# GuanLab/seekmer

Measured on AMD Instinct MI355X. Metric: paired reads/sec mapped+quantified, higher is better.
Workload: dtype u64+f64; 1 GPU; configs[1]: synthetic ~190k-tx index (stand-in for ENSEMBL GRCh38 cDNA), 10000000 2x100bp synthetic pairs per GPU, map+classes+EM to the reference stop rule; transcripts=190402, kmer_slots=134217728, units_per_gpu=10000000, read_len=100, paired=True, classes=851072, class_map_rows=4208693, parallelism=reads sharded x1, RCCL all-reduce f64[T] per EM step, rccl_ranks=0

## Files before the change

### seekmer_amd/csrc/skm_abi.hip

```cpp
#include "../../include/seekmer_hip.h"
#include "skm_kernels.h"
#include "skm_pool.h"

#include <dlfcn.h>
#include <algorithm>
#include <cstdarg>
#include <cstdio>
#include <cstdlib>
#include <cstring>
#include <chrono>
#include <condition_variable>
#include <atomic>
#include <deque>
#include <functional>
#include <map>
#include <memory>
#include <unordered_map>
#include <mutex>
#include <thread>
#include <numeric>
#include <string>
#include <utility>
#include <vector>

// ... 218 lines not shown
struct skm_quant {
    ~skm_quant()
    {
        (void)hipSetDevice(device);
        if (stream) (void)hipStreamSynchronize(stream);
    }
    int device = 0;
    PoolStream stream;
    PoolTimingEvent ev[2];
    PoolEvent chunk_ev[2];
    PoolPinned pinned;
    std::mutex mu;
    int64_t n_tx = 0, n_classes = 0, n_ids = 0, n_rows = 0;
    DBuf<int64_t> cls_offset, row_start, tx_row;
    DBuf<int32_t> ids, tx_cls, row_tx, perm;
    DBuf<double> cls_count, cls_count_saved, inner, row_sum;
    DBuf<double> eff_len, x0, x1, acc, part_max;
    DBuf<unsigned int> part_flags, arrivals;
    DBuf<unsigned long long> ctl, cum;
    DBuf<unsigned int> tile_total;
    DBuf<double> x_start, boot_out;
    struct Batch {
        DBuf<double> cls_count, inner, row_sum, x0, x1, part_max;
        DBuf<unsigned int> part_flags;
        DBuf<unsigned long long> ctl, mgr;
        DBuf<double> counts_all;
        DBuf<double> totals;
        DBuf<int64_t> iters;
    } batch;
    struct Tiles {
        DBuf<int64_t> tile_tx, tile_cls, cls_pair, tx_pair;
        DBuf<int32_t> tx_list, cls_list, tx_label, tx_tile, cls_tile;
        DBuf<uint16_t> cls_tx, tx_cls;
        DBuf<double> x2, step_max;
        DBuf<unsigned int> step_flags;
        struct Residual {
            int64_t n_classes = 0, n_ids = 0, n_rows = 0;
            DBuf<int64_t> cls_offset, row_start, tx_row;
            DBuf<int32_t> ids, cls_src, row_tx, tx_cls;
            DBuf<double> cls_count, inner, row_sum;
            bool built = false;
        } residual;
        bool built = false;
        int64_t n_tiles = 0, n_oversize = 0;
    } tiles;
    double n_total = 0;
    bool n_total_reduced = false;
    void *comm = nullptr;
    int rank = 0, world = 1;
    double t_em_ns = 0, iters_total = 0, launches = 0;
};

struct skm_comm {
    int device = 0;
    void *comm = nullptr;
    int rank = 0, world = 1;
};

extern "C" const char *skm_last_error(void) { return g_error.c_str(); }

extern "C" int skm_device_count(int *count)
{
    if (!count) return fail(SKM_ERR_ARG, "count is NULL");
    int n = 0;
    hipError_t e = hipGetDeviceCount(&n);
    if (e != hipSuccess || n <= 0) {
        *count = 0;
// ... 2233 lines not shown
    HIP_TRY(pool_stream_acquire(q->stream.out()));
    for (auto &e : q->ev) HIP_TRY(pool_event_acquire(e.out(), true));
    for (auto &e : q->chunk_ev) HIP_TRY(pool_event_acquire(e.out(), false));
    HIP_TRY(pool_pinned_acquire((void **)q->pinned.out()));
    const size_t C = (size_t)std::max<int64_t>(n_classes, 1), M = (size_t)std::max<int64_t>(n_ids, 1);
    const size_t T = (size_t)std::max<int64_t>(n_tx, 1);
    const size_t R = (size_t)quant_rows_upper_bound(n_tx, n_ids);
    SKM_TRY(q->cls_offset.ensure(C + 1));
    SKM_TRY(q->cls_count.ensure(C));
    SKM_TRY(q->inner.ensure(C));
    SKM_TRY(q->ids.ensure(M));
    SKM_TRY(q->perm.ensure(C));
    SKM_TRY(q->tx_cls.ensure(M));
    SKM_TRY(q->tx_row.ensure(T + 1));
    SKM_TRY(q->row_start.ensure(R + 1));
    SKM_TRY(q->row_tx.ensure(R));
    SKM_TRY(q->row_sum.ensure(R));
    SKM_TRY(q->eff_len.ensure(T));
    SKM_TRY(q->x0.ensure(T));
    SKM_TRY(q->x1.ensure(T));
    SKM_TRY(q->acc.ensure(T));
    SKM_TRY(q->ctl.ensure(16));
    SKM_TRY(q->part_max.ensure(EM_FINAL_BLOCKS));
    SKM_TRY(q->part_flags.ensure(EM_FINAL_BLOCKS));
    SKM_TRY(q->arrivals.ensure(T));
    HIP_TRY(hipMemsetAsync(q->arrivals.p, 0, T * sizeof(unsigned int), q->stream));
    if (em_tiles_possible(several_ranks)) {
        auto &t = q->tiles;
        SKM_TRY(t.tile_tx.ensure(T + 2)); SKM_TRY(t.tile_cls.ensure(T + 2));
        SKM_TRY(t.cls_pair.ensure(C + 1)); SKM_TRY(t.tx_pair.ensure(T + 1));
        SKM_TRY(t.tx_list.ensure(T)); SKM_TRY(t.cls_list.ensure(C));
        SKM_TRY(t.tx_label.ensure(T)); SKM_TRY(t.tx_tile.ensure(T)); SKM_TRY(t.cls_tile.ensure(C));
        SKM_TRY(t.cls_tx.ensure(M)); SKM_TRY(t.tx_cls.ensure(M));
        SKM_TRY(t.x2.ensure(T));
    }
    STALE_CHECK("quant_alloc exit");
    return SKM_OK;
}

QuantBuild quant_build_view(skm_quant *q)
{
    QuantBuild b{};
    b.n_tx = q->n_tx;
    b.n_classes = q->n_classes;
    b.n_ids = q->n_ids;
    b.cls_offset = q->cls_offset.p;
    b.ids = q->ids.p;
    b.cls_count = q->cls_count.p;
    b.tx_cls = q->tx_cls.p;
    b.tx_row = q->tx_row.p;
    b.row_start = q->row_start.p;
    b.row_tx = q->row_tx.p;
    b.n_rows_cap = (int64_t)q->row_tx.cap;
    if (q->tiles.x2.p) {
        auto &t = q->tiles;
        b.tile_tx = t.tile_tx.p; b.tile_cls = t.tile_cls.p;
        b.tx_list = t.tx_list.p; b.cls_list = t.cls_list.p;
        b.cls_pair = t.cls_pair.p; b.tx_pair = t.tx_pair.p;
        b.tile_cls_tx = t.cls_tx.p; b.tile_tx_cls = t.tx_cls.p;
        b.tx_label = t.tx_label.p; b.tx_tile = t.tx_tile.p; b.cls_tile = t.cls_tile.p;
    }
    return b;
}

int quant_finish_setup(skm_quant *q, const ClassTable *table, int64_t units_seen = -1)
{
    STALE_CHECK("quant_finish_setup");
    QuantBuild b = quant_build_view(q);
    b.first_seen_bound = units_seen > 0 ? units_seen : 0;
    const int64_t rows = quant_setup(table, b, q->perm.p, q->stream);
    if (rows < 0) return fail(SKM_ERR_HIP, "building the class views failed (%lld): %s", (long long)rows, quant_setup_failure());
    q->n_rows = rows;
    if (b.tile_tx) {
        q->tiles.built = true;
        q->tiles.n_tiles = b.tile_info[0];
        q->tiles.n_oversize = b.tile_info[1];
        if (q->tiles.n_tiles > 0) {
            SKM_TRY(q->tiles.step_max.ensure((size_t)(EM_CHUNK_MAX * q->tiles.n_tiles)));
            SKM_TRY(q->tiles.step_flags.ensure((size_t)(EM_CHUNK_MAX * q->tiles.n_tiles)));
        }
        if (q->tiles.n_oversize > 0 && q->tiles.n_tiles > 0) {
            auto &r = q->tiles.residual;
            int64_t counts[3] = {0, 0, 0};
            if (quant_residual_count(b, counts, q->stream))
                return fail(SKM_ERR_HIP, "sizing the residual EM problem failed: %s", quant_setup_failure());
            r.n_classes = counts[0]; r.n_ids = counts[1]; r.n_rows = counts[2];
            SKM_TRY(r.cls_offset.ensure((size_t)r.n_classes + 1)); SKM_TRY(r.ids.ensure((size_t)std::max<int64_t>(r.n_ids, 1)));
            SKM_TRY(r.cls_src.ensure((size_t)std::max<int64_t>(r.n_classes, 1)));
            SKM_TRY(r.row_start.ensure((size_t)r.n_rows + 1)); SKM_TRY(r.row_tx.ensure((size_t)std::max<int64_t>(r.n_rows, 1)));
            SKM_TRY(r.tx_cls.ensure((size_t)std::max<int64_t>(r.n_ids, 1))); SKM_TRY(r.tx_row.ensure((size_t)q->n_tx + 1));
            SKM_TRY(r.cls_count.ensure((size_t)std::max<int64_t>(r.n_classes, 1)));
            SKM_TRY(r.inner.ensure((size_t)std::max<int64_t>(r.n_classes, 1)));
            SKM_TRY(r.row_sum.ensure((size_t)std::max<int64_t>(r.n_rows, 1)));
            QuantResidual out{};
            out.n_classes = r.n_classes; out.n_ids = r.n_ids; out.n_rows = r.n_rows;
            out.cls_offset = r.cls_offset.p; out.ids = r.ids.p; out.cls_src = r.cls_src.p;
            out.row_start = r.row_start.p; out.row_tx = r.row_tx.p; out.tx_cls = r.tx_cls.p; out.tx_row = r.tx_row.p;
            if (quant_residual_build(b, out, q->stream))
                return fail(SKM_ERR_HIP, "building the residual EM problem failed: %s", quant_setup_failure());
            r.built = true;
        }
    }
    return SKM_OK;
}

struct Rccl {
    void *lib = nullptr;
    int (*GetUniqueId)(void *) = nullptr;
    int (*AllReduce)(const void *, void *, size_t, int, int, void *, hipStream_t) = nullptr;
    int (*CommDestroy)(void *) = nullptr;
    int (*CommCount)(void *, int *) = nullptr;
    const char *(*GetErrorString)(int) = nullptr;
// ... 61 lines not shown
    p.x[1] = q->x1.p;
    p.acc = q->acc.p;
    p.n_total = q->n_total;
    p.rel_tol = rel_tol;
    p.x_floor = x_floor;
    p.ctl = q->ctl.p;
    p.part_max = q->part_max.p;
    p.part_flags = q->part_flags.p;
    p.max_iters = max_iters;
    p.fixed_iters = fixed_iters;
    static const bool unfused = getenv("SKM_EM_UNFUSED") != nullptr;
    p.fused = q->comm || unfused ? 0 : 1;
    p.arrivals = q->arrivals.p;
    return p;
}

bool em_uses_tiles(const skm_quant *q)
{
    return em_tiles_possible(q->comm != nullptr) && q->tiles.built && q->tiles.n_tiles > 0 &&
           (q->tiles.n_oversize == 0 || q->tiles.residual.built);
}

constexpr int CTL_WORD_TILE_FAULT = 4;
int em_run_tiles(skm_quant *q, const EmProblem &p, int64_t chunk, int64_t *iters_out)
{
    auto &t = q->tiles;
    EmTiles tl{};
    tl.n_tiles = t.n_tiles;
    tl.tile_tx = t.tile_tx.p; tl.tile_cls = t.tile_cls.p;
    tl.tx_list = t.tx_list.p; tl.cls_list = t.cls_list.p;
    tl.cls_pair = t.cls_pair.p; tl.tx_pair = t.tx_pair.p;
    tl.cls_tx = t.cls_tx.p; tl.tx_cls = t.tx_cls.p;
    tl.step_max = t.step_max.p; tl.step_flags = t.step_flags.p;
    double *const x[3] = {q->x0.p, q->x1.p, t.x2.p};
    const bool mixed = t.n_oversize > 0;
    EmProblem pr = p;
    if (mixed) {
        auto &r = t.residual;
        pr.n_classes = r.n_classes; pr.n_rows = r.n_rows;
        pr.cls_offset = r.cls_offset.p; pr.ids = r.ids.p; pr.cls_count = r.cls_count.p; pr.inner = r.inner.p;
        pr.row_start = r.row_start.p; pr.row_tx = r.row_tx.p; pr.tx_cls = r.tx_cls.p; pr.tx_row = r.tx_row.p;
        pr.row_sum = r.row_sum.p;
        pr.fused = 1;
        pr.extra_max = t.step_max.p; pr.extra_flags = t.step_flags.p; pr.n_extra = t.n_tiles;
        launch_permute_f64(q->cls_count.p, r.cls_src.p, r.n_classes, r.cls_count.p, false, q->stream);
    }
    int64_t queued = 0;
    auto enqueue_chunk = [&](int slot) -> int {
        launch_em_local_chunk(p, tl, x[queued % 3], x[(queued + 1) % 3], (int)chunk, true, q->stream);
        if (mixed) {
            pr.extra_first = queued * chunk;
            for (int64_t i = 0, k = queued * chunk; i < chunk; ++i, ++k) {
                launch_em_inner(pr, (int)(k & 1), i > 0, k, q->stream);
                launch_em_rows_finalize(pr, (int)(k & 1), q->stream);
            }
            launch_em_decide(pr, (queued + 1) * chunk, q->stream);
            q->launches += 2 * chunk + 2;
        } else {
            launch_em_local_decide(p, tl, queued * chunk, (int)chunk, q->stream);
            q->launches += 2;
        }
        ++queued;
        HIP_TRY(hipGetLastError());
        HIP_TRY(hipMemcpyAsync(q->pinned + 8 * slot, q->ctl.p, 8 * sizeof(unsigned long long),
                               hipMemcpyDeviceToHost, q->stream));
        HIP_TRY(hipEventRecord(q->chunk_ev[slot], q->stream));
        return SKM_OK;
    };
    unsigned long long ctl[8] = {0};
    SKM_TRY(enqueue_chunk(0));
    int64_t last = 0;
    for (int slot = 0;; slot ^= 1, ++last) {
        SKM_TRY(enqueue_chunk(slot ^ 1));
        HIP_TRY(hipEventSynchronize(q->chunk_ev[slot]));
        memcpy(ctl, q->pinned + 8 * slot, sizeof(ctl));
        if (ctl[0]) break;
    }
    if (ctl[CTL_WORD_TILE_FAULT]) {
        HIP_TRY(hipStreamSynchronize(q->stream));
        return fail(SKM_ERR_STATE, "a component tile exceeds the tile capacity: the class views of this handle are damaged");
    }
    const int64_t steps = (int64_t)ctl[1], into = steps - last * chunk;
    double *const result = (steps & 1) ? q->x1.p : q->x0.p;
    if (into == chunk && !mixed) {
        if (x[(last + 1) % 3] != result)
            HIP_TRY(hipMemcpyAsync(result, x[(last + 1) % 3], q->n_tx * 8, hipMemcpyDeviceToDevice, q->stream));
    } else {
        launch_em_local_chunk(p, tl, x[last % 3], result, (int)into, false, q->stream);
        q->launches += 1;
        HIP_TRY(hipGetLastError());
    }
    HIP_TRY(hipEventRecord(q->ev[1], q->stream));
    HIP_TRY(hipEventSynchronize(q->ev[1]));
    float ms = 0;
    HIP_TRY(hipEventElapsedTime(&ms, q->ev[0], q->ev[1]));
    q->t_em_ns += ms * 1e6;
    q->iters_total += (double)steps;
    if (iters_out) *iters_out = steps;
    if (ctl[3]) return fail(SKM_ERR_UNDEFINED, "no abundance above x_floor: numpy raises on max() of an empty selection");
    return SKM_OK;
}

int em_run(skm_quant *q, double rel_tol, double x_floor, int64_t max_iters, int64_t fixed_iters,
           int64_t *iters_out, int64_t chunk_steps = 16)
{
    double n_total = q->n_total;
    if (q->comm && !q->n_total_reduced) {
        HIP_TRY(hipMemcpyAsync(q->acc.p, &n_total, 8, hipMemcpyHostToDevice, q->stream));
        NCCL_TRY(g_rccl.AllReduce(q->acc.p, q->acc.p, 1, NCCL_FLOAT64, NCCL_SUM, q->comm, q->stream));
        HIP_TRY(hipMemcpyAsync(&n_total, q->acc.p, 8, hipMemcpyDeviceToHost, q->stream));
        HIP_TRY(hipStreamSynchronize(q->stream));
    }
    EmProblem p = em_problem(q, rel_tol, x_floor, max_iters, fixed_iters);
    p.n_total = n_total;
    HIP_TRY(hipMemsetAsync(q->ctl.p, 0, 16 * 8, q->stream));
    int64_t k = 0;
    const int64_t chunk = fixed_iters > 0 ? std::min<int64_t>(fixed_iters, chunk_steps) : chunk_steps;
    HIP_TRY(hipEventRecord(q->ev[0], q->stream));
    if (em_uses_tiles(q) && chunk <= EM_CHUNK_MAX) return em_run_tiles(q, p, chunk, iters_out);
    static const bool unfused_rows = getenv("SKM_EM_UNFUSED") != nullptr;
    auto enqueue_chunk = [&](int slot) -> int {
        for (int64_t i = 0; i < chunk; ++i, ++k) {
            launch_em_inner(p, (int)(k & 1), i > 0, k, q->stream);
            if (q->comm) {
// ... 778 lines not shown
```

### seekmer_amd/csrc/skm_em.hip

```cpp
#include "skm_kernels.h"

namespace skm {

enum { CTL_DONE = 0, CTL_ITERS = 1, CTL_UNDEFINED = 3, CTL_TILE_FAULT = 4 };

__device__ bool em_evaluate(const EmProblem &p, int n_parts, int64_t steps_done, bool publish);

__global__ void __launch_bounds__(256)
em_inner_kernel(EmProblem p, int parity, int eval_parts, int64_t steps_done)
{
    const int64_t c_first = blockIdx.x * (int64_t)blockDim.x + threadIdx.x;
    int64_t begin_first = 0, end_first = 0;
    double count_first = 1.0;
    if (c_first < p.n_classes) {
        begin_first = p.cls_offset[c_first];
        end_first = p.cls_offset[c_first + 1];
        count_first = p.cls_count[c_first];
    }
    if (eval_parts > 0 && blockIdx.x == 0) {
        if (p.ctl[CTL_DONE]) return;
        if (em_evaluate(p, eval_parts, steps_done, true)) return;
    } else if (p.ctl[CTL_DONE]) {
        return;
    }
// ... 223 lines not shown
    const int wave = threadIdx.x >> 6;
    if ((threadIdx.x & 63) == 0) { s_max[wave] = m; s_flags[wave] = f; }
    __syncthreads();
    if (threadIdx.x == 0) {
        for (int w = 0; w < 4; ++w) { m = s_max[w] > m ? s_max[w] : m; f |= s_flags[w]; }
        bool done, undefined = false;
        if (p.fixed_iters > 0) {
            done = steps_done >= p.fixed_iters;
        } else if (!(f & 1u)) {
            undefined = true;
            done = true;
        } else {
            done = (f & 2u) || !(m > p.rel_tol);
            if (p.max_iters > 0 && steps_done >= p.max_iters) done = true;
        }
        if (publish) {
            if (undefined) p.ctl[CTL_UNDEFINED] = 1;
            p.ctl[CTL_ITERS] = (unsigned long long)steps_done;
            p.ctl[CTL_DONE] = done ? 1ULL : 0ULL;
        }
        s_done = done ? 1 : 0;
    }
    __syncthreads();
    return s_done != 0;
}

__global__ void __launch_bounds__(256)
em_decide_kernel(EmProblem p, int n_parts, int64_t steps_done)
{
    if (p.ctl[CTL_DONE]) return;
    em_evaluate(p, n_parts, steps_done, true);
}

__global__ void __launch_bounds__(256)
em_local_chunk_kernel(EmProblem p, EmTiles tl, const double *x_in, double *x_out, int n_steps, int check_done)
{
    static_assert(EM_TILE_TX <= 8 * 32, "a lane group of the row phase takes at most eight transcripts");
    if (check_done && p.ctl[CTL_DONE]) return;
    __shared__ double s_x[2][EM_TILE_TX];
    __shared__ double s_eff[EM_TILE_TX];
    __shared__ double s_inner[EM_TILE_CLASSES];
    __shared__ double s_count[EM_TILE_CLASSES];
    __shared__ double s_max[EM_CHUNK_MAX][4];
    __shared__ unsigned int s_flags[EM_CHUNK_MAX][4];
    __shared__ int32_t s_tx[EM_TILE_TX];
    __shared__ uint16_t s_cls_tx[EM_TILE_PAIRS], s_tx_cls[EM_TILE_PAIRS];
    __shared__ uint16_t s_cls_off[EM_TILE_CLASSES + 1], s_tx_off[EM_TILE_TX + 1];
    const int64_t tile = blockIdx.x;
    const int64_t tx0 = tl.tile_tx[tile], cls0 = tl.tile_cls[tile];
    const int n_tx = (int)(tl.tile_tx[tile + 1] - tx0), n_cls = (int)(tl.tile_cls[tile + 1] - cls0);
    const int64_t cp0 = tl.cls_pair[cls0], tp0 = tl.tx_pair[tx0];
    const int n_pairs = (int)(tl.cls_pair[cls0 + n_cls] - cp0);
    if (n_tx > EM_TILE_TX || n_cls > EM_TILE_CLASSES || n_pairs > EM_TILE_PAIRS || n_tx < 0 || n_cls < 0 || n_pairs < 0) {
        if (threadIdx.x == 0) { p.ctl[CTL_TILE_FAULT] = 1; p.ctl[CTL_DONE] = 1; }
        return;
    }
    const int tid = threadIdx.x;
    for (int j = tid; j < n_pairs; j += 256) {
        s_cls_tx[j] = tl.cls_tx[cp0 + j];
        s_tx_cls[j] = tl.tx_cls[tp0 + j];
    }
    for (int k = tid; k <= n_cls; k += 256) {
        s_cls_off[k] = (uint16_t)(tl.cls_pair[cls0 + k] - cp0);
        if (k < n_cls) s_count[k] = p.cls_count[tl.cls_list[cls0 + k]];
    }
    for (int i = tid; i <= n_tx; i += 256) {
        s_tx_off[i] = (uint16_t)(tl.tx_pair[tx0 + i] - tp0);
        if (i < n_tx) {
            const int32_t t = tl.tx_list[tx0 + i];
            s_tx[i] = t;
            s_x[0][i] = x_in[t];
            s_eff[i] = p.eff_len[t];
        }
    }
    __syncthreads();
    const int sub = tid & 7, wave = tid >> 6;
    for (int step = 0; step < n_steps; ++step) {
        const double *x = s_x[step & 1];
        double *x_new = s_x[(step & 1) ^ 1];
        for (int k = tid; k < n_cls; k += 256) {
            const int end = s_cls_off[k + 1];
            double s = 0.0;
            for (int j = s_cls_off[k]; j < end; ++j) s += x[s_cls_tx[j]];
            s_inner[k] = s / s_count[k];
        }
        __syncthreads();
        double local_max = 0.0;
        unsigned int flags = 0;
        double my_a = 0.0, my_xt = 0.0;
        int my_i = -1, turn = 0;
        for (int i = tid >> 3; i < n_tx; i += 32, ++turn) {
            const double xt = x[i];
            const int end = s_tx_off[i + 1];
            int begin = s_tx_off[i];
            double a = 0.0;
            do {
                const int row_end = min(begin + EM_ROW_CAP, end);
                double s = 0.0;
                for (int e = begin + sub; e < row_end; e += 8) s += xt / s_inner[s_tx_cls[e]];
                s += __shfl_xor(s, 4, 8);
                s += __shfl_xor(s, 2, 8);
                s += __shfl_xor(s, 1, 8);
                a += s;
                begin = row_end;
            } while (begin < end);
            if (turn == sub) { my_a = a; my_xt = xt; my_i = i; }
        }
        if (my_i >= 0) {
            double v = my_a / s_eff[my_i] / p.n_total;
            if (v != v) v = 0.0;
            x_new[my_i] = v;
            if (v > p.x_floor) {
                const double change = fabs(v - my_xt) / v;
                if (change != change) flags |= 2u;
                else if (change > local_max) local_max = change;
                flags |= 1u;
            }
        }
        for (int d = 32; d > 0; d >>= 1) {
            const double o = __shfl_xor(local_max, d, 64);
            local_max = o > local_max ? o : local_max;
            flags |= __shfl_xor(flags, d, 64);
        }
        if ((tid & 63) == 0) { s_max[step][wave] = local_max; s_flags[step][wave] = flags; }
        __syncthreads();
    }
    const double *x = s_x[n_steps & 1];
    for (int i = tid; i < n_tx; i += 256) x_out[s_tx[i]] = x[i];
    if (tid < n_steps) {
        double m = s_max[tid][0];
        unsigned int f = s_flags[tid][0];
        for (int w = 1; w < 4; ++w) { m = s_max[tid][w] > m ? s_max[tid][w] : m; f |= s_flags[tid][w]; }
        tl.step_max[tid * tl.n_tiles + tile] = m;
        tl.step_flags[tid * tl.n_tiles + tile] = f;
    }
}

__global__ void __launch_bounds__(64 * EM_CHUNK_MAX)
em_local_decide_kernel(EmProblem p, EmTiles tl, int64_t first_step, int n_steps)
{
    if (p.ctl[CTL_DONE]) return;
    __shared__ double s_max[EM_CHUNK_MAX];
    __shared__ unsigned int s_flags[EM_CHUNK_MAX];
    const int step = threadIdx.x >> 6, lane = threadIdx.x & 63;
    if (step < n_steps) {
        double m = 0.0;
        unsigned int f = 0;
        const double *__restrict__ step_max = tl.step_max + step * tl.n_tiles;
        const unsigned int *__restrict__ step_flags = tl.step_flags + step * tl.n_tiles;
        int64_t b = lane;
        for (; b + 7 * 64 < tl.n_tiles; b += 8 * 64) {
            double o[8];
            unsigned int g[8];
#pragma unroll
            for (int k = 0; k < 8; ++k) { o[k] = step_max[b + 64 * k]; g[k] = step_flags[b + 64 * k]; }
#pragma unroll
            for (int k = 0; k < 8; ++k) { m = o[k] > m ? o[k] : m; f |= g[k]; }
        }
        for (; b < tl.n_tiles; b += 64) {
            const double o = step_max[b];
            m = o > m ? o : m;
// ... 277 lines not shown
    if (blocks < 1) blocks = 1;
    if (blocks > EM_FINAL_BLOCKS) blocks = EM_FINAL_BLOCKS;
    return (int)blocks;
}

void launch_em_inner(const EmProblem &p, int parity, bool judge_previous, int64_t steps_done, hipStream_t stream)
{
    hipLaunchKernelGGL(em_inner_kernel, dim3(chip_grid(p.n_classes, 256)), dim3(256), 0, stream, p, parity,
                       judge_previous ? em_final_blocks(p) : 0, steps_done);
}

void launch_em_decide(const EmProblem &p, int64_t steps_done, hipStream_t stream)
{
    hipLaunchKernelGGL(em_decide_kernel, dim3(1), dim3(256), 0, stream, p, em_final_blocks(p), steps_done);
}

void launch_em_rows(const EmProblem &p, int parity, hipStream_t stream)
{
    hipLaunchKernelGGL(em_rows_kernel, dim3(chip_grid(p.n_rows, 32)), dim3(256), 0, stream, p, parity);
}

void launch_em_rows_finalize(const EmProblem &p, int parity, hipStream_t stream)
{
    hipLaunchKernelGGL(em_rows_finalize_kernel<false>, dim3((unsigned)em_final_blocks(p)), dim3(256), 0, stream, p, parity);
}

void launch_em_rows_acc(const EmProblem &p, int parity, hipStream_t stream)
{
    EmProblem fused = p;
    fused.fused = 1;
    hipLaunchKernelGGL(em_rows_finalize_kernel<true>, dim3((unsigned)em_final_blocks(fused)), dim3(256), 0, stream, p, parity);
}

void launch_em_local_chunk(const EmProblem &p, const EmTiles &tiles, const double *x_in, double *x_out, int n_steps,
                           bool check_done, hipStream_t stream)
{
    if (tiles.n_tiles <= 0 || n_steps <= 0) return;
    hipLaunchKernelGGL(em_local_chunk_kernel, dim3((unsigned)tiles.n_tiles), dim3(256), 0, stream, p, tiles, x_in, x_out,
                       std::min(n_steps, EM_CHUNK_MAX), check_done ? 1 : 0);
}

void launch_em_local_decide(const EmProblem &p, const EmTiles &tiles, int64_t first_step, int n_steps, hipStream_t stream)
{
    hipLaunchKernelGGL(em_local_decide_kernel, dim3(1), dim3(64 * EM_CHUNK_MAX), 0, stream, p, tiles, first_step,
                       std::min(n_steps, EM_CHUNK_MAX));
}

void launch_em_rows_to_acc(const EmProblem &p, hipStream_t stream)
{
    hipLaunchKernelGGL(em_rows_to_acc_kernel, dim3(chip_grid(p.n_tx, 256)), dim3(256), 0, stream, p);
}

void launch_em_finalize(const EmProblem &p, int parity, bool from_acc, hipStream_t stream)
{
    const int blocks = em_final_blocks(p);
    if (from_acc)
        hipLaunchKernelGGL(em_finalize_kernel<true>, dim3((unsigned)blocks), dim3(256), 0, stream, p, parity);
    else
        hipLaunchKernelGGL(em_finalize_kernel<false>, dim3((unsigned)blocks), dim3(256), 0, stream, p, parity);
}

constexpr int NP_MAX_LEAVES = 160;

__device__ __forceinline__ double np_leaf_sum(const double *a, int n)
{
    if (n < 8) {
        double r = 0.0;
        for (int i = 0; i < n; ++i) r += a[i];
        return r;
    }
    double r[8];
    for (int j = 0; j < 8; ++j) r[j] = a[j];
// ... 277 lines not shown
```

### seekmer_amd/csrc/skm_kernels.h

```cpp
#pragma once
#include "skm_device.h"

namespace skm {

struct MapBatch {
    const uint32_t *records;
    int64_t n_units;
    int32_t words_per_read;
    int32_t record_words;
    int32_t paired;
    int32_t *workspace;
    int32_t *rec_unit;
    uint64_t *rec_key;
    unsigned long long *rec_tuple;
    int32_t keep_spans;
    int32_t *unit_begin, *unit_end;
    Coord *unit_anchor;
    int32_t *unit_entries;
    int64_t ids_capacity;
    unsigned long long *ids_cursor;
    unsigned long long *fld;
    unsigned long long *stats;
    int32_t vote[8];
};
// ... 128 lines not shown
    const int32_t *tx_cls;
    const int64_t *tx_row;
    double *row_sum;
    const double *eff_len;
    double *x[2];
    double *acc;
    double n_total;
    double rel_tol, x_floor;
    unsigned long long *ctl;
    double *part_max;
    unsigned int *part_flags;
    int64_t max_iters, fixed_iters;
    int fused;
    unsigned int *arrivals;
    const double *extra_max;
    const unsigned int *extra_flags;
    int64_t n_extra, extra_first;
};
#ifndef SKM_EM_FINAL_BLOCKS
#define SKM_EM_FINAL_BLOCKS 2048
#endif
constexpr int EM_FINAL_BLOCKS = SKM_EM_FINAL_BLOCKS;
void launch_em_inner(const EmProblem &p, int parity, bool judge_previous, int64_t steps_done, hipStream_t stream);
void launch_em_decide(const EmProblem &p, int64_t steps_done, hipStream_t stream);
void launch_em_rows(const EmProblem &p, int parity, hipStream_t stream);
void launch_em_rows_finalize(const EmProblem &p, int parity, hipStream_t stream);
void launch_em_rows_acc(const EmProblem &p, int parity, hipStream_t stream);
void launch_em_rows_to_acc(const EmProblem &p, hipStream_t stream);
void launch_em_finalize(const EmProblem &p, int parity, bool from_acc, hipStream_t stream);
void launch_em_result(const unsigned long long *ctl, const double *x0, const double *x1, int64_t n, double *out,
                      hipStream_t stream);

constexpr int EM_TILE_PAIRS = 2048, EM_TILE_CLASSES = 512, EM_TILE_TX = 128;
constexpr int EM_TILE_SEGMENT = 128;
constexpr int EM_CHUNK_MAX = 16;
struct EmTiles {
    int64_t n_tiles;
    const int64_t *tile_tx;
    const int64_t *tile_cls;
    const int32_t *tx_list;
    const int32_t *cls_list;
    const int64_t *cls_pair;
    const int64_t *tx_pair;
    const uint16_t *cls_tx;
    const uint16_t *tx_cls;
    double *step_max;
    unsigned int *step_flags;
};
void launch_em_local_chunk(const EmProblem &p, const EmTiles &tiles, const double *x_in, double *x_out, int n_steps,
                           bool check_done, hipStream_t stream);
void launch_em_local_decide(const EmProblem &p, const EmTiles &tiles, int64_t first_step, int n_steps, hipStream_t stream);

constexpr int EM_BATCH = 8;
struct EmBatchProblem {
    int64_t n_tx, n_classes, n_rows;
    const int64_t *cls_offset;
    const int32_t *ids;
    const int64_t *row_start;
    const int32_t *row_tx;
    const int32_t *tx_cls;
    const int64_t *tx_row;
    const double *eff_len;
    const double *cls_count;
    double *inner;
    double *row_sum;
    double *x[2];
    double *place_total;
    double rel_tol, x_floor;
    unsigned long long *ctl;
    double *part_max;
    unsigned int *part_flags;
    int managed;
    unsigned long long *mgr;
    int64_t *iters_out;
    int fused;
    unsigned int *arrivals;
};
void launch_em_batch_manage_init(const EmBatchProblem &p, unsigned long long *mgr, unsigned long long *host_pinned64,
                                 int64_t n_reps, const double *counts_all, const double *totals, const double *x_start,
                                 double *out_all, hipStream_t stream);
void launch_em_batch_manage(const EmBatchProblem &p, unsigned long long *mgr, const double *counts_all, const double *totals,
                            const double *x_start, double *out_all, int64_t *iters_out, int64_t step, bool planned,
                            hipStream_t stream);
// ... 67 lines not shown
```

### seekmer_amd/csrc/skm_quant_setup.hip

```cpp
#include "skm_kernels.h"
#include "skm_pool.h"

#include <algorithm>
#include <cstdio>
#include <vector>

namespace skm {

namespace {

struct Scratch {
    hipStream_t stream;
    std::vector<void *> held;
    explicit Scratch(hipStream_t s) : stream(s) {}
    template <class T>
    T *alloc(size_t n)
    {
        void *p = nullptr;
        if (pool_alloc(&p, std::max<size_t>(n, 1) * sizeof(T)) != hipSuccess) return nullptr;
        held.push_back(p);
        return static_cast<T *>(p);
    }
    ~Scratch()
    {
// ... 746 lines not shown
                if (c_tx > EM_TILE_TX || c_pairs > EM_TILE_PAIRS || c_classes > EM_TILE_CLASSES) {
                    root_tile[t] = -2;
                    atomicAdd(oversize, 1ULL);
                    continue;
                }
                if (n == 0 || tx + c_tx > EM_TILE_TX || pairs + c_pairs > EM_TILE_PAIRS ||
                    classes + c_classes > EM_TILE_CLASSES) {
                    ++n;
                    tx = pairs = classes = 0;
                }
                tx += c_tx; pairs += c_pairs; classes += c_classes;
                root_tile[t] = n - 1;
            }
        }
        seg_tiles[g] = n;
    }
}

__global__ void __launch_bounds__(256)
tx_tile_kernel(const int32_t *label, const int32_t *root_tile, const int64_t *seg_base, int64_t n_tx,
               const int64_t *tx_row, const int64_t *row_start, int degree_bits, int32_t *tx_tile, int32_t *key)
{
    for (int64_t t = blockIdx.x * (int64_t)blockDim.x + threadIdx.x; t < n_tx;
         t += (int64_t)gridDim.x * blockDim.x) {
        const int32_t r = label[t], at = root_tile[r];
        const int32_t tile = at < 0 ? (int32_t)n_tx : (int32_t)(seg_base[r / EM_TILE_SEGMENT] + at);
        tx_tile[t] = tile;
        const int64_t turns = (row_start[tx_row[t + 1]] - row_start[tx_row[t]] + 7) >> 3;
        const int32_t longest = (1 << degree_bits) - 1;
        key[t] = (tile << degree_bits) | (longest - (int32_t)min(turns, (int64_t)longest));
    }
}

__global__ void __launch_bounds__(256)
cls_tile_kernel(const int64_t *cls_offset, const int32_t *ids, int64_t n_classes, const int32_t *tx_tile,
                int32_t *cls_tile)
{
    for (int64_t c = blockIdx.x * (int64_t)blockDim.x + threadIdx.x; c < n_classes;
         c += (int64_t)gridDim.x * blockDim.x) {
        const int64_t begin = cls_offset[c];
        cls_tile[c] = tx_tile[begin < cls_offset[c + 1] ? ids[begin] : 0];
    }
}

__global__ void __launch_bounds__(256)
tile_starts_kernel(const int32_t *sorted_tile, int shift, int64_t n, const int64_t *n_tiles, int64_t *first)
{
    const int64_t tiles = *n_tiles;
    for (int64_t j = blockIdx.x * (int64_t)blockDim.x + threadIdx.x; j <= n;
         j += (int64_t)gridDim.x * blockDim.x) {
        const int64_t lo = j == 0 ? -1 : min((int64_t)(sorted_tile[j - 1] >> shift), tiles);
        const int64_t hi = j == n ? tiles : min((int64_t)(sorted_tile[j] >> shift), tiles);
        for (int64_t t = lo + 1; t <= hi; ++t) first[t] = j;
    }
}

__global__ void __launch_bounds__(256)
tile_local_tx_kernel(const int32_t *list, const int32_t *tile_sorted, int shift, const int64_t *first, const int64_t *n_tiles, int64_t n,
                     const int64_t *tx_row, const int64_t *row_start, int32_t *local, int64_t *len)
{
    for (int64_t i = blockIdx.x * (int64_t)blockDim.x + threadIdx.x; i < n;
         i += (int64_t)gridDim.x * blockDim.x) {
        const int32_t t = list[i];
        local[t] = (int32_t)(i - first[min((int64_t)(tile_sorted[i] >> shift), *n_tiles)]);
        len[i] = row_start[tx_row[t + 1]] - row_start[tx_row[t]];
    }
}

__global__ void __launch_bounds__(256)
tile_local_cls_kernel(const int32_t *list, const int32_t *tile_sorted, const int64_t *first, const int64_t *n_tiles, int64_t n,
                      const int64_t *cls_offset, int32_t *local, int64_t *len)
{
    for (int64_t k = blockIdx.x * (int64_t)blockDim.x + threadIdx.x; k < n;
         k += (int64_t)gridDim.x * blockDim.x) {
        const int32_t c = list[k];
        local[c] = (int32_t)(k - first[min((int64_t)tile_sorted[k], *n_tiles)]);
        len[k] = cls_offset[c + 1] - cls_offset[c];
    }
}

__global__ void __launch_bounds__(256)
tile_fill_cls_kernel(const int32_t *cls_list, int64_t n_classes, const int64_t *cls_offset, const int32_t *ids,
                     const int32_t *tx_local, const int64_t *cls_pair, const int32_t *cls_tile, int32_t residual_tile,
                     uint16_t *out)
{
    for (int64_t k = blockIdx.x * (int64_t)blockDim.x + threadIdx.x; k < n_classes;
         k += (int64_t)gridDim.x * blockDim.x) {
        const int32_t c = cls_list[k];
        if (cls_tile[c] == residual_tile) continue;
        const int64_t src = cls_offset[c], n = cls_offset[c + 1] - src, dst = cls_pair[k];
        for (int64_t j = 0; j < n; ++j) out[dst + j] = (uint16_t)tx_local[ids[src + j]];
    }
}

__global__ void __launch_bounds__(256)
tile_fill_tx_kernel(const int32_t *tx_list, int64_t n_tx, const int64_t *tx_row, const int64_t *row_start,
                    const int32_t *tx_cls, const int32_t *cls_local, const int64_t *tx_pair, const int32_t *tx_tile,
                    uint16_t *out)
{
    const int sub = threadIdx.x & 7;
    for (int64_t i = (blockIdx.x * (int64_t)blockDim.x + threadIdx.x) >> 3; i < n_tx;
         i += ((int64_t)gridDim.x * blockDim.x) >> 3) {
        const int32_t t = tx_list[i];
        if (tx_tile[t] == (int32_t)n_tx) continue;
        const int64_t src = row_start[tx_row[t]], n = row_start[tx_row[t + 1]] - src, dst = tx_pair[i];
        for (int64_t j = sub; j < n; j += 8) out[dst + j] = (uint16_t)cls_local[tx_cls[src + j]];
    }
}

// ... 3 lines not shown
    const int64_t C = q.n_classes, M = q.n_ids, T = q.n_tx;
    if (M >= (1LL << 31) || C >= (1LL << 31) || T >= (1LL << 31) - 2) return -2;
    const int64_t n_segments = (T + EM_TILE_SEGMENT - 1) / EM_TILE_SEGMENT;
    QB_ALLOC(parent, int32_t, T); QB_ALLOC(comp, int32_t, 3 * T); QB_ALLOC(root_tile, int32_t, T);
    QB_ALLOC(seg_tiles, int64_t, n_segments); QB_ALLOC(seg_base, int64_t, n_segments + 1);
    QB_ALLOC(oversize, unsigned long long, 1);
    QB_ALLOC(iota, int32_t, std::max(T, C)); QB_ALLOC(sorted_tile, int32_t, std::max(T, C));
    QB_ALLOC(tx_local, int32_t, T); QB_ALLOC(cls_local, int32_t, C);
    QB_ALLOC(len, int64_t, std::max(T, C));
    QB_TRY(hipMemsetAsync(comp, 0, 3 * T * sizeof(int32_t), stream));
    QB_TRY(hipMemsetAsync(oversize, 0, sizeof(unsigned long long), stream));
    hipLaunchKernelGGL(iota_kernel, dim3(blocks_for(T)), dim3(256), 0, stream, parent, T);
    hipLaunchKernelGGL(cc_hook_kernel, dim3(blocks_for(C)), dim3(256), 0, stream, q.cls_offset, q.ids, C, parent);
    hipLaunchKernelGGL(cc_label_kernel, dim3(blocks_for(T)), dim3(256), 0, stream, parent, q.tx_row, q.row_start, T,
                       q.tx_label, comp);
    hipLaunchKernelGGL(cc_classes_kernel, dim3(blocks_for(C)), dim3(256), 0, stream, q.cls_offset, q.ids, C,
                       q.tx_label, comp);
    hipLaunchKernelGGL(tile_pack_kernel, dim3(blocks_for(n_segments)), dim3(256), 0, stream, comp, T, n_segments,
                       root_tile, seg_tiles, oversize);
    if (exclusive_scan_with_total(scratch, seg_tiles, seg_base, n_segments)) return -1;
    int end_bit = 1;
    while ((1LL << end_bit) < T + 1 && end_bit < 31) ++end_bit;
    const int degree_bits = end_bit + 5 <= 31 ? 5 : 0;
    QB_ALLOC(tx_key, int32_t, T);
    hipLaunchKernelGGL(tx_tile_kernel, dim3(blocks_for(T)), dim3(256), 0, stream, q.tx_label, root_tile, seg_base, T,
                       q.tx_row, q.row_start, degree_bits, q.tx_tile, tx_key);
    hipLaunchKernelGGL(iota_kernel, dim3(blocks_for(std::max(T, C))), dim3(256), 0, stream, iota, std::max(T, C));
    if (sort_pairs(scratch, tx_key, sorted_tile, iota, q.tx_list, T, end_bit + degree_bits)) return -1;
    hipLaunchKernelGGL(tile_starts_kernel, dim3(blocks_for(T + 1)), dim3(256), 0, stream, sorted_tile, degree_bits, T,
                       seg_base + n_segments, q.tile_tx);
    hipLaunchKernelGGL(tile_local_tx_kernel, dim3(blocks_for(T)), dim3(256), 0, stream, q.tx_list, sorted_tile, degree_bits,
                       q.tile_tx, seg_base + n_segments, T, q.tx_row, q.row_start, tx_local, len);
    if (exclusive_scan_with_total(scratch, len, q.tx_pair, T)) return -1;
    hipLaunchKernelGGL(cls_tile_kernel, dim3(blocks_for(C)), dim3(256), 0, stream, q.cls_offset, q.ids, C, q.tx_tile,
                       q.cls_tile);
    if (sort_pairs(scratch, q.cls_tile, sorted_tile, iota, q.cls_list, C, end_bit)) return -1;
    hipLaunchKernelGGL(tile_starts_kernel, dim3(blocks_for(C + 1)), dim3(256), 0, stream, sorted_tile, 0, C,
                       seg_base + n_segments, q.tile_cls);
    hipLaunchKernelGGL(tile_local_cls_kernel, dim3(blocks_for(C)), dim3(256), 0, stream, q.cls_list, sorted_tile,
                       q.tile_cls, seg_base + n_segments, C, q.cls_offset, cls_local, len);
    if (exclusive_scan_with_total(scratch, len, q.cls_pair, C)) return -1;
    hipLaunchKernelGGL(tile_fill_cls_kernel, dim3(blocks_for(C)), dim3(256), 0, stream, q.cls_list, C, q.cls_offset,
                       q.ids, tx_local, q.cls_pair, q.cls_tile, (int32_t)T, q.tile_cls_tx);
    hipLaunchKernelGGL(tile_fill_tx_kernel, dim3(blocks_for(8 * T)), dim3(256), 0, stream, q.tx_list, T, q.tx_row,
                       q.row_start, q.tx_cls, cls_local, q.tx_pair, q.tx_tile, q.tile_tx_cls);
    QB_TRY(hipMemcpyAsync(&q.tile_info[0], seg_base + n_segments, sizeof(int64_t), hipMemcpyDeviceToHost, stream));
    QB_TRY(hipMemcpyAsync(&q.tile_info[1], oversize, sizeof(int64_t), hipMemcpyDeviceToHost, stream));
    return 0;
}

}

int64_t quant_setup(const ClassTable *table, QuantBuild &q, int32_t *perm, hipStream_t stream)
{
    const bool can_rank = table && q.first_seen_bound > 0 && q.first_seen_bound <= RANK_BITMAP_MAX_UNITS;
    for (int attempt = can_rank ? 0 : 1; attempt < 2; ++attempt) {
        int64_t n_rows = -1;
        {
            Scratch scratch(stream);
            if (attempt == 0) {
                const int rc = build_from_table_ranked(scratch, *table, q, perm);
                if (rc == 1) continue;
                if (rc) return -1;
            } else {
                if (table && build_from_table(scratch, *table, q)) return -1;
                if (localize(scratch, q, perm)) return -1;
            }
            if (transpose(scratch, q)) return -1;
            if (q.tile_tx && build_tiles(scratch, q)) return -1;
            QB_TRY(hipGetLastError());
            QB_TRY(hipMemcpyAsync(&n_rows, q.tx_row + q.n_tx, sizeof(int64_t), hipMemcpyDeviceToHost, stream));
        }
// ... 127 lines not shown
```

Baseline: 952.5 million pairs/s.

## Snapshot per-step EM tile states and drop the final recompute chunk

The tiled EM chunk kernel now writes every step's transcript abundances into a per-step snapshot buffer. Once convergence is flagged, the next launched chunk copies the converged step's values out of that buffer instead of the host launching a trailing partial chunk or a device copy. This removes the triple x buffer rotation and the extra synchronised relaunch at the end. The class inner-sum loop also gathers four entries per turn, and the set-up sorts classes within a tile by length to balance lanes. The cost is an extra global write per transcript per step and a buffer of EM_CHUNK_MAX times T doubles.

```diff
diff --git a/seekmer_amd/csrc/skm_abi.hip b/seekmer_amd/csrc/skm_abi.hip
--- a/seekmer_amd/csrc/skm_abi.hip
+++ b/seekmer_amd/csrc/skm_abi.hip
@@ -274,7 +274,7 @@
         DBuf<int64_t> tile_tx, tile_cls, cls_pair, tx_pair;
         DBuf<int32_t> tx_list, cls_list, tx_label, tx_tile, cls_tile;
         DBuf<uint16_t> cls_tx, tx_cls;
-        DBuf<double> x2, step_max;
+        DBuf<double> snap, step_max;
         DBuf<unsigned int> step_flags;
         struct Residual {
             int64_t n_classes = 0, n_ids = 0, n_rows = 0;
@@ -2574,7 +2574,6 @@
         SKM_TRY(t.tx_list.ensure(T)); SKM_TRY(t.cls_list.ensure(C));
         SKM_TRY(t.tx_label.ensure(T)); SKM_TRY(t.tx_tile.ensure(T)); SKM_TRY(t.cls_tile.ensure(C));
         SKM_TRY(t.cls_tx.ensure(M)); SKM_TRY(t.tx_cls.ensure(M));
-        SKM_TRY(t.x2.ensure(T));
     }
     STALE_CHECK("quant_alloc exit");
     return SKM_OK;
@@ -2594,7 +2593,7 @@
     b.row_start = q->row_start.p;
     b.row_tx = q->row_tx.p;
     b.n_rows_cap = (int64_t)q->row_tx.cap;
-    if (q->tiles.x2.p) {
+    if (q->tiles.tile_tx.p) {
         auto &t = q->tiles;
         b.tile_tx = t.tile_tx.p; b.tile_cls = t.tile_cls.p;
         b.tx_list = t.tx_list.p; b.cls_list = t.cls_list.p;
@@ -2620,6 +2619,7 @@
         if (q->tiles.n_tiles > 0) {
             SKM_TRY(q->tiles.step_max.ensure((size_t)(EM_CHUNK_MAX * q->tiles.n_tiles)));
             SKM_TRY(q->tiles.step_flags.ensure((size_t)(EM_CHUNK_MAX * q->tiles.n_tiles)));
+            SKM_TRY(q->tiles.snap.ensure((size_t)EM_CHUNK_MAX * (size_t)q->n_tx));
         }
         if (q->tiles.n_oversize > 0 && q->tiles.n_tiles > 0) {
             auto &r = q->tiles.residual;
@@ -2747,7 +2747,7 @@
     tl.cls_pair = t.cls_pair.p; tl.tx_pair = t.tx_pair.p;
     tl.cls_tx = t.cls_tx.p; tl.tx_cls = t.tx_cls.p;
     tl.step_max = t.step_max.p; tl.step_flags = t.step_flags.p;
-    double *const x[3] = {q->x0.p, q->x1.p, t.x2.p};
+    tl.snap = t.snap.p;
     const bool mixed = t.n_oversize > 0;
     EmProblem pr = p;
     if (mixed) {
@@ -2762,7 +2762,7 @@
     }
     int64_t queued = 0;
     auto enqueue_chunk = [&](int slot) -> int {
-        launch_em_local_chunk(p, tl, x[queued % 3], x[(queued + 1) % 3], (int)chunk, true, q->stream);
+        launch_em_local_chunk(p, tl, queued == 0 ? q->x0.p : t.snap.p + (chunk - 1) * q->n_tx, (int)chunk, queued * chunk, q->stream);
         if (mixed) {
             pr.extra_first = queued * chunk;
             for (int64_t i = 0, k = queued * chunk; i < chunk; ++i, ++k) {
@@ -2784,8 +2784,7 @@
     };
     unsigned long long ctl[8] = {0};
     SKM_TRY(enqueue_chunk(0));
-    int64_t last = 0;
-    for (int slot = 0;; slot ^= 1, ++last) {
+    for (int slot = 0;; slot ^= 1) {
         SKM_TRY(enqueue_chunk(slot ^ 1));
         HIP_TRY(hipEventSynchronize(q->chunk_ev[slot]));
         memcpy(ctl, q->pinned + 8 * slot, sizeof(ctl));
@@ -2795,16 +2794,7 @@
         HIP_TRY(hipStreamSynchronize(q->stream));
         return fail(SKM_ERR_STATE, "a component tile exceeds the tile capacity: the class views of this handle are damaged");
     }
-    const int64_t steps = (int64_t)ctl[1], into = steps - last * chunk;
-    double *const result = (steps & 1) ? q->x1.p : q->x0.p;
-    if (into == chunk && !mixed) {
-        if (x[(last + 1) % 3] != result)
-            HIP_TRY(hipMemcpyAsync(result, x[(last + 1) % 3], q->n_tx * 8, hipMemcpyDeviceToDevice, q->stream));
-    } else {
-        launch_em_local_chunk(p, tl, x[last % 3], result, (int)into, false, q->stream);
-        q->launches += 1;
-        HIP_TRY(hipGetLastError());
-    }
+    const int64_t steps = (int64_t)ctl[1];
     HIP_TRY(hipEventRecord(q->ev[1], q->stream));
     HIP_TRY(hipEventSynchronize(q->ev[1]));
     float ms = 0;
diff --git a/seekmer_amd/csrc/skm_em.hip b/seekmer_amd/csrc/skm_em.hip
--- a/seekmer_amd/csrc/skm_em.hip
+++ b/seekmer_amd/csrc/skm_em.hip
@@ -279,11 +279,19 @@
     em_evaluate(p, n_parts, steps_done, true);
 }
 
-__global__ void __launch_bounds__(256)
-em_local_chunk_kernel(EmProblem p, EmTiles tl, const double *x_in, double *x_out, int n_steps, int check_done)
+#ifndef SKM_EM_TILE_EXPERIMENT
+#define SKM_EM_TILE_EXPERIMENT 0
+#endif
+#ifndef SKM_EM_CLASS_BATCH
+#define SKM_EM_CLASS_BATCH 4
+#endif
+constexpr int EM_CLASS_BATCH = SKM_EM_CLASS_BATCH;
+static_assert(EM_CLASS_BATCH == EM_TILE_CLASS_BATCH || EM_CLASS_BATCH == 1, "the set-up orders classes by turns of this width");
+
+__global__ void __launch_bounds__(256)
+em_local_chunk_kernel(EmProblem p, EmTiles tl, const double *x_in, int n_steps, int64_t first_step)
 {
     static_assert(EM_TILE_TX <= 8 * 32, "a lane group of the row phase takes at most eight transcripts");
-    if (check_done && p.ctl[CTL_DONE]) return;
     __shared__ double s_x[2][EM_TILE_TX];
     __shared__ double s_eff[EM_TILE_TX];
     __shared__ double s_inner[EM_TILE_CLASSES];
@@ -303,6 +311,17 @@
         return;
     }
     const int tid = threadIdx.x;
+    if (p.ctl[CTL_DONE]) {
+        const int64_t steps = (int64_t)p.ctl[CTL_ITERS], at = steps - 1 - (first_step - n_steps);
+        if (p.ctl[CTL_TILE_FAULT] || first_step < n_steps || at < 0 || at >= n_steps) return;
+        const double *__restrict__ from = tl.snap + at * p.n_tx;
+        double *__restrict__ to = p.x[steps & 1];
+        for (int i = tid; i < n_tx; i += 256) {
+            const int32_t t = tl.tx_list[tx0 + i];
+            to[t] = from[t];
+        }
+        return;
+    }
     for (int j = tid; j < n_pairs; j += 256) {
         s_cls_tx[j] = tl.cls_tx[cp0 + j];
         s_tx_cls[j] = tl.tx_cls[tp0 + j];
@@ -310,6 +329,7 @@
     for (int k = tid; k <= n_cls; k += 256) {
         s_cls_off[k] = (uint16_t)(tl.cls_pair[cls0 + k] - cp0);
         if (k < n_cls) s_count[k] = p.cls_count[tl.cls_list[cls0 + k]];
+        if ((SKM_EM_TILE_EXPERIMENT & 1) && k < n_cls) s_inner[k] = 1.0;
     }
     for (int i = tid; i <= n_tx; i += 256) {
         s_tx_off[i] = (uint16_t)(tl.tx_pair[tx0 + i] - tp0);
@@ -325,38 +345,60 @@
     for (int step = 0; step < n_steps; ++step) {
         const double *x = s_x[step & 1];
         double *x_new = s_x[(step & 1) ^ 1];
-        for (int k = tid; k < n_cls; k += 256) {
-            const int end = s_cls_off[k + 1];
-            double s = 0.0;
-            for (int j = s_cls_off[k]; j < end; ++j) s += x[s_cls_tx[j]];
-            s_inner[k] = s / s_count[k];
+        if (!(SKM_EM_TILE_EXPERIMENT & 1)) {
+            for (int k = tid; k < n_cls; k += 256) {
+                const int end = s_cls_off[k + 1];
+                double s = 0.0;
+                if (EM_CLASS_BATCH == 1) {
+                    for (int j = s_cls_off[k]; j < end; ++j) s += x[s_cls_tx[j]];
+                } else {
+                    for (int j = s_cls_off[k]; j < end; j += EM_CLASS_BATCH) {
+                        int t[EM_CLASS_BATCH];
+                        double v[EM_CLASS_BATCH];
+#pragma unroll
+                        for (int b = 0; b < EM_CLASS_BATCH; ++b) t[b] = s_cls_tx[min(j + b, end - 1)];
+#pragma unroll
+                        for (int b = 0; b < EM_CLASS_BATCH; ++b) v[b] = x[t[b]];
+                        s += v[0];
+#pragma unroll
+                        for (int b = 1; b < EM_CLASS_BATCH; ++b) {
+                            const double with = s + v[b];
+                            s = j + b < end ? with : s;
+                        }
+                    }
+                }
+                s_inner[k] = s / s_count[k];
+            }
         }
         __syncthreads();
         double local_max = 0.0;
         unsigned int flags = 0;
         double my_a = 0.0, my_xt = 0.0;
         int my_i = -1, turn = 0;
-        for (int i = tid >> 3; i < n_tx; i += 32, ++turn) {
-            const double xt = x[i];
-            const int end = s_tx_off[i + 1];
-            int begin = s_tx_off[i];
-            double a = 0.0;
-            do {
-                const int row_end = min(begin + EM_ROW_CAP, end);
-                double s = 0.0;
-                for (int e = begin + sub; e < row_end; e += 8) s += xt / s_inner[s_tx_cls[e]];
-                s += __shfl_xor(s, 4, 8);
-                s += __shfl_xor(s, 2, 8);
-                s += __shfl_xor(s, 1, 8);
-                a += s;
-                begin = row_end;
-            } while (begin < end);
-            if (turn == sub) { my_a = a; my_xt = xt; my_i = i; }
+        if (!(SKM_EM_TILE_EXPERIMENT & 2)) {
+            for (int i = tid >> 3; i < n_tx; i += 32, ++turn) {
+                const double xt = x[i];
+                const int end = s_tx_off[i + 1];
+                int begin = s_tx_off[i];
+                double a = 0.0;
+                do {
+                    const int row_end = min(begin + EM_ROW_CAP, end);
+                    double s = 0.0;
+                    for (int e = begin + sub; e < row_end; e += 8) s += xt / s_inner[s_tx_cls[e]];
+                    s += __shfl_xor(s, 4, 8);
+                    s += __shfl_xor(s, 2, 8);
+                    s += __shfl_xor(s, 1, 8);
+                    a += s;
+                    begin = row_end;
+                } while (begin < end);
+                if (turn == sub) { my_a = a; my_xt = xt; my_i = i; }
+            }
         }
         if (my_i >= 0) {
             double v = my_a / s_eff[my_i] / p.n_total;
             if (v != v) v = 0.0;
             x_new[my_i] = v;
+            tl.snap[step * p.n_tx + s_tx[my_i]] = v;
             if (v > p.x_floor) {
                 const double change = fabs(v - my_xt) / v;
                 if (change != change) flags |= 2u;
@@ -372,8 +414,6 @@
         if ((tid & 63) == 0) { s_max[step][wave] = local_max; s_flags[step][wave] = flags; }
         __syncthreads();
     }
-    const double *x = s_x[n_steps & 1];
-    for (int i = tid; i < n_tx; i += 256) x_out[s_tx[i]] = x[i];
     if (tid < n_steps) {
         double m = s_max[tid][0];
         unsigned int f = s_flags[tid][0];
@@ -717,12 +757,12 @@
     hipLaunchKernelGGL(em_rows_finalize_kernel<true>, dim3((unsigned)em_final_blocks(fused)), dim3(256), 0, stream, p, parity);
 }
 
-void launch_em_local_chunk(const EmProblem &p, const EmTiles &tiles, const double *x_in, double *x_out, int n_steps,
-                           bool check_done, hipStream_t stream)
+void launch_em_local_chunk(const EmProblem &p, const EmTiles &tiles, const double *x_in, int n_steps, int64_t first_step,
+                           hipStream_t stream)
 {
     if (tiles.n_tiles <= 0 || n_steps <= 0) return;
-    hipLaunchKernelGGL(em_local_chunk_kernel, dim3((unsigned)tiles.n_tiles), dim3(256), 0, stream, p, tiles, x_in, x_out,
-                       std::min(n_steps, EM_CHUNK_MAX), check_done ? 1 : 0);
+    hipLaunchKernelGGL(em_local_chunk_kernel, dim3((unsigned)tiles.n_tiles), dim3(256), 0, stream, p, tiles, x_in,
+                       std::min(n_steps, EM_CHUNK_MAX), first_step);
 }
 
 void launch_em_local_decide(const EmProblem &p, const EmTiles &tiles, int64_t first_step, int n_steps, hipStream_t stream)
diff --git a/seekmer_amd/csrc/skm_kernels.h b/seekmer_amd/csrc/skm_kernels.h
--- a/seekmer_amd/csrc/skm_kernels.h
+++ b/seekmer_amd/csrc/skm_kernels.h
@@ -184,8 +184,12 @@
                       hipStream_t stream);
 
 constexpr int EM_TILE_PAIRS = 2048, EM_TILE_CLASSES = 512, EM_TILE_TX = 128;
-constexpr int EM_TILE_SEGMENT = 128;
+#ifndef SKM_EM_TILE_SEGMENT
+#define SKM_EM_TILE_SEGMENT 128
+#endif
+constexpr int EM_TILE_SEGMENT = SKM_EM_TILE_SEGMENT;
 constexpr int EM_CHUNK_MAX = 16;
+constexpr int EM_TILE_CLASS_BATCH = 4;
 struct EmTiles {
     int64_t n_tiles;
     const int64_t *tile_tx;
@@ -198,9 +202,10 @@
     const uint16_t *tx_cls;
     double *step_max;
     unsigned int *step_flags;
-};
-void launch_em_local_chunk(const EmProblem &p, const EmTiles &tiles, const double *x_in, double *x_out, int n_steps,
-                           bool check_done, hipStream_t stream);
+    double *snap;
+};
+void launch_em_local_chunk(const EmProblem &p, const EmTiles &tiles, const double *x_in, int n_steps, int64_t first_step,
+                           hipStream_t stream);
 void launch_em_local_decide(const EmProblem &p, const EmTiles &tiles, int64_t first_step, int n_steps, hipStream_t stream);
 
 constexpr int EM_BATCH = 8;
diff --git a/seekmer_amd/csrc/skm_quant_setup.hip b/seekmer_amd/csrc/skm_quant_setup.hip
--- a/seekmer_amd/csrc/skm_quant_setup.hip
+++ b/seekmer_amd/csrc/skm_quant_setup.hip
@@ -802,14 +802,21 @@
     }
 }
 
+#ifndef SKM_EM_CLASS_ORDER
+#define SKM_EM_CLASS_ORDER 1
+#endif
 __global__ void __launch_bounds__(256)
 cls_tile_kernel(const int64_t *cls_offset, const int32_t *ids, int64_t n_classes, const int32_t *tx_tile,
-                int32_t *cls_tile)
+                int length_bits, int32_t *cls_tile, int32_t *key)
 {
     for (int64_t c = blockIdx.x * (int64_t)blockDim.x + threadIdx.x; c < n_classes;
          c += (int64_t)gridDim.x * blockDim.x) {
-        const int64_t begin = cls_offset[c];
-        cls_tile[c] = tx_tile[begin < cls_offset[c + 1] ? ids[begin] : 0];
+        const int64_t begin = cls_offset[c], end = cls_offset[c + 1];
+        const int32_t tile = tx_tile[begin < end ? ids[begin] : 0];
+        cls_tile[c] = tile;
+        const int64_t turns = (end - begin + EM_TILE_CLASS_BATCH - 1) / EM_TILE_CLASS_BATCH;
+        const int32_t longest = (1 << length_bits) - 1;
+        key[c] = (tile << length_bits) | (longest - (int32_t)min(turns, (int64_t)longest));
     }
 }
 
@@ -838,13 +845,13 @@
 }
 
 __global__ void __launch_bounds__(256)
-tile_local_cls_kernel(const int32_t *list, const int32_t *tile_sorted, const int64_t *first, const int64_t *n_tiles, int64_t n,
+tile_local_cls_kernel(const int32_t *list, const int32_t *tile_sorted, int shift, const int64_t *first, const int64_t *n_tiles, int64_t n,
                       const int64_t *cls_offset, int32_t *local, int64_t *len)
 {
     for (int64_t k = blockIdx.x * (int64_t)blockDim.x + threadIdx.x; k < n;
          k += (int64_t)gridDim.x * blockDim.x) {
         const int32_t c = list[k];
-        local[c] = (int32_t)(k - first[min((int64_t)tile_sorted[k], *n_tiles)]);
+        local[c] = (int32_t)(k - first[min((int64_t)(tile_sorted[k] >> shift), *n_tiles)]);
         len[k] = cls_offset[c + 1] - cls_offset[c];
     }
 }
@@ -914,12 +921,14 @@
     hipLaunchKernelGGL(tile_local_tx_kernel, dim3(blocks_for(T)), dim3(256), 0, stream, q.tx_list, sorted_tile, degree_bits,
                        q.tile_tx, seg_base + n_segments, T, q.tx_row, q.row_start, tx_local, len);
     if (exclusive_scan_with_total(scratch, len, q.tx_pair, T)) return -1;
+    const int length_bits = SKM_EM_CLASS_ORDER ? degree_bits : 0;
+    QB_ALLOC(cls_key, int32_t, C);
     hipLaunchKernelGGL(cls_tile_kernel, dim3(blocks_for(C)), dim3(256), 0, stream, q.cls_offset, q.ids, C, q.tx_tile,
-                       q.cls_tile);
-    if (sort_pairs(scratch, q.cls_tile, sorted_tile, iota, q.cls_list, C, end_bit)) return -1;
-    hipLaunchKernelGGL(tile_starts_kernel, dim3(blocks_for(C + 1)), dim3(256), 0, stream, sorted_tile, 0, C,
+                       length_bits, q.cls_tile, cls_key);
+    if (sort_pairs(scratch, cls_key, sorted_tile, iota, q.cls_list, C, end_bit + length_bits)) return -1;
+    hipLaunchKernelGGL(tile_starts_kernel, dim3(blocks_for(C + 1)), dim3(256), 0, stream, sorted_tile, length_bits, C,
                        seg_base + n_segments, q.tile_cls);
-    hipLaunchKernelGGL(tile_local_cls_kernel, dim3(blocks_for(C)), dim3(256), 0, stream, q.cls_list, sorted_tile,
+    hipLaunchKernelGGL(tile_local_cls_kernel, dim3(blocks_for(C)), dim3(256), 0, stream, q.cls_list, sorted_tile, length_bits,
                        q.tile_cls, seg_base + n_segments, C, q.cls_offset, cls_local, len);
     if (exclusive_scan_with_total(scratch, len, q.cls_pair, C)) return -1;
     hipLaunchKernelGGL(tile_fill_cls_kernel, dim3(blocks_for(C)), dim3(256), 0, stream, q.cls_list, C, q.cls_offset,
```

New measurement: 971.7 million pairs/s, median of 6. 2.0% higher.
